# smcconoughey/erpl_monte_carlo_sim

Measured on AMD Instinct MI355X. Metric: Monte Carlo trajectories/sec (whole node) + apogee-match rate, higher is better.
Workload: dtype f64_fast

## Files before the change

erpl_monte_carlo_sim_amd/csrc/erpl_k_config.h:

```cpp
#pragma once

#ifndef ERPL_FAITHFUL
#define ERPL_FAITHFUL 0
#endif
#ifndef ERPL_FAST_F64
#define ERPL_FAST_F64 0
#endif
#ifndef ERPL_FAST_F32
#define ERPL_FAST_F32 0
#endif
#if ERPL_FAITHFUL + ERPL_FAST_F64 + ERPL_FAST_F32 != 1
#error "define exactly one of ERPL_FAITHFUL, ERPL_FAST_F64, ERPL_FAST_F32 to 1 before including erpl_kernels.inc"
#endif

#define ERPL_CAT_(a, b) a##b
#define ERPL_CAT(a, b) ERPL_CAT_(a, b)
#if ERPL_FAITHFUL
typedef double real;
#define ERPL_SUFFIX f64
#elif ERPL_FAST_F64
typedef double real;
#define ERPL_SUFFIX f64f
#else
typedef float real;
#define ERPL_SUFFIX f32
#endif
#define ERPL_LAUNCH_NAME ERPL_CAT(erpl_launch_, ERPL_SUFFIX)

#ifndef ERPL_STAGE_UNROLL
#if ERPL_FAITHFUL
#define ERPL_STAGE_UNROLL 1
#else
#define ERPL_STAGE_UNROLL 4
#endif
#endif
#ifndef ERPL_FLIGHT_MIN_WAVES
#if ERPL_FAITHFUL
#define ERPL_FLIGHT_MIN_WAVES 1
#else
#define ERPL_FLIGHT_MIN_WAVES 2
#endif
#endif
#ifndef ERPL_DENSE_WAVES
#define ERPL_DENSE_WAVES 3
#endif
#ifndef ERPL_SWEEP_CAPPED_WAVES
#define ERPL_SWEEP_CAPPED_WAVES 2
#endif
#ifndef ERPL_RAIL_BLOCK
#define ERPL_RAIL_BLOCK 64
#endif
#ifndef ERPL_HANDOFF_SPEED
#define ERPL_HANDOFF_SPEED 1e6
#endif

#ifndef ERPL_STAMPS
#define ERPL_STAMPS 0
#endif
#if ERPL_STAMPS
#define ERPL_STAMP(acc_, last_)                                                          \
  do {                                                                                   \
    __builtin_amdgcn_sched_barrier(0);                                                   \
    unsigned long long now_;                                                             \
    asm volatile("s_memtime %0\n\ts_waitcnt lgkmcnt(0)" : "=s"(now_)::"memory");          \
    __builtin_amdgcn_sched_barrier(0);                                                   \
    acc_ += now_ - last_;                                                                \
    last_ = now_;                                                                        \
  } while (0)
#else
#define ERPL_STAMP(acc_, last_) do { } while (0)
#endif

namespace {
constexpr bool kFaithful = (ERPL_FAITHFUL != 0);
constexpr int kWave = 64;
struct StampSums { unsigned long long seg[8]; unsigned long long last; };
}
#define ERPL_RARE_BLOCK() asm volatile("")
```

erpl_monte_carlo_sim_amd/csrc/erpl_k_debug.h:

```cpp
namespace {

#if ERPL_FAITHFUL
struct RecordEval {
  real mass, cg, Ixx, Iyy;
  real T, P, rho;
  real vb0, vb1, vb2, vn, mach;
  real alpha, beta;
  real cd, cl, cy, cm, cyaw, cp_dyn;
  real qdyn, thrust, drag, margin;
};
__device__ __forceinline__ void record_eval(const Shared& C, const LaneParams& p, int64_t id, double ts,
                                            const real (&y)[14], RecordEval& e) {
  const ErplScalars<real>& S = *C.S;
  mass_props(S, p, y[13], e.mass, e.cg, e.Ixx, e.Iyy);
  atmosphere(S, y[2], e.T, e.P);
  e.rho = e.P / (S.Rg * e.T);
  WindCache wc;
  wc.lo = 1; wc.hi = 0; wc.x0 = 0;
#pragma unroll
  for (int c = 0; c < 3; ++c) { wc.y0[c] = 0; wc.s[c] = 0; }
  real wv[3];
  wind_at(C, id, y[2], wc, wv);
  const real vr0 = y[3] - wv[0], vr1 = y[4] - wv[1], vr2 = y[5] - wv[2];
  real w = y[6], x = y[7], yy = y[8], z = y[9];
// ... 29 lines not shown
}

__device__ __forceinline__ void lane_params_of(const ErplKArgs& a, const ErplScalars<real>& S, int64_t id, LaneParams& p) {
  const int64_t n = a.n;
  p.dry = (real)a.rocket[0 * n + id]; p.prop = (real)a.rocket[1 * n + id];
  p.thrust = (real)a.motor[0 * n + id]; p.Ae = (real)a.motor[1 * n + id];
  p.mdot = (real)a.motor[2 * n + id]; p.burn = a.motor[3 * n + id];
  lane_params_finish(S, p);
}

__global__ __launch_bounds__(256) void erpl_extract_f64(const ErplKArgs a, const ErplScalars<real> S,
                                                        const double time_offset) {
  __shared__ LdsTables L;
  __shared__ real alt_s[ERPL_MAX_WIND_KNOTS];
  stage_tables(L, alt_s, a.tables, a.alt_grid, a.k_wind);
  const int64_t r = (int64_t)blockIdx.x * blockDim.x + threadIdx.x;
  if (r >= a.traj_cap) return;
  Shared C;
  C.S = &S; C.L = &L; C.alt = alt_s; C.has_wind = a.k_wind > 0; C.motor_kind = a.motor_kind;
  const int64_t id = a.n_traj;
  LaneParams p;
  lane_params_of(a, S, id, p);
  const double* rec = a.traj + r * ERPL_TRAJ_DIM;
  const double ts = rec[0] - time_offset;
  real y[14];
#pragma unroll
  for (int c = 0; c < 14; ++c) y[c] = (real)rec[1 + c];
  double* o = a.summary + r * ERPL_DIAG_DIM;
  {
    const real w = y[6], x = y[7], yy = y[8], z = y[9];
    o[0] = atan2(2 * (w * x + yy * z), 1 - 2 * (x * x + yy * yy));
    const real sinp = 2 * (w * yy - z * x);
    o[1] = (fabs(sinp) >= 1) ? copysign(1.57079632679489661923, sinp) : asin(sinp);
    o[2] = atan2(2 * (w * z + x * yy), 1 - 2 * (yy * yy + z * z));
  }
  RecordEval e;
  record_eval(C, p, id, ts, y, e);
  o[3] = e.cg; o[4] = e.mass; o[5] = e.Ixx; o[6] = e.Iyy; o[7] = e.Iyy;
  o[8] = e.thrust;
  o[9] = e.drag;
  o[10] = e.cd; o[11] = e.cl; o[12] = e.cm;
  o[13] = e.cp_dyn;
  o[14] = e.margin;
  o[15] = e.alpha; o[16] = e.beta;
}
#endif

__global__ __launch_bounds__(256) void ERPL_CAT(erpl_debug_, ERPL_SUFFIX)(const ErplKArgs a, const ErplScalars<real> S,
                                                                         const int what, const int64_t m,
                                                                         const double* __restrict__ in,
                                                                         double* __restrict__ out) {
  __shared__ LdsTables L;
  __shared__ real alt_s[ERPL_MAX_WIND_KNOTS];
  stage_tables(L, alt_s, a.tables, a.alt_grid, a.k_wind);
  const int64_t j = (int64_t)blockIdx.x * blockDim.x + threadIdx.x;
  const int64_t n = a.n;
  if (j >= ((what == ERPL_DBG_RHS_SEQ) ? n : m)) return;
  Shared C;
  C.S = &S; C.L = &L; C.alt = alt_s; C.has_wind = a.k_wind > 0; C.motor_kind = a.motor_kind;
  const int64_t id = j % n;
  LaneParams p;
  p.dry = (real)a.rocket[0 * n + id]; p.prop = (real)a.rocket[1 * n + id];
  p.thrust = (real)a.motor[0 * n + id]; p.Ae = (real)a.motor[1 * n + id];
  p.mdot = (real)a.motor[2 * n + id]; p.burn = a.motor[3 * n + id];
  lane_params_finish(S, p);
  WindCache wc;
  wc.lo = 1; wc.hi = 0; wc.x0 = 0;
#pragma unroll
  for (int c = 0; c < 3; ++c) { wc.y0[c] = 0; wc.s[c] = 0; }
  MachCache mc;
  mach_cache_clear(mc);
  AtmCache ac;
  atm_cache_clear(ac);
#if !ERPL_FAITHFUL
  LaneRec lr;
#if ERPL_FAST_F64
  __shared__ real lane_wind[kLwSlots][kWave];
  lr.lw = &lane_wind[0][threadIdx.x];
  lr.put_wind(wc);
#endif
#endif
  if (what == ERPL_DBG_ATMOSPHERE) {
    const real h = (real)in[j];
    real T, P, rho, g;
#if ERPL_FAITHFUL
    atmosphere(S, h, T, P);
    rho = m_div(P, S.Rg * T);
    g = gravity_at(S, h);
#else
    real rT;
    altitude_tables_reload(C, id, h, wc, ac);
    fast_atmosphere(C, ac, h, T, rT, P);
    rho = (P * S.inv_Rg) * rT;
    const real re = (real)6.371e6;
    const real r = re * m_rcp(re + h);
    g = S.g0 * (r * r);
#endif
    out[0 * m + j] = (double)T; out[1 * m + j] = (double)P; out[2 * m + j] = (double)rho; out[3 * m + j] = (double)g;
  } else if (what == ERPL_DBG_AERO) {
    const real mach = (real)in[0 * m + j], alpha = (real)in[1 * m + j], beta = (real)in[2 * m + j];
    const real pf = (real)in[3 * m + j];
    mach_lookup(C, mach, mc);
    real cd, cl, cy, cm, cyaw;
#if ERPL_FAITHFUL
    real mass, cg, Ixx, Iyy, cp_dyn;
    mass_props(S, p, pf, mass, cg, Ixx, Iyy);
    aero_coefficients(S, mach_rec_of(C, mc), mach, alpha, beta, cg, in[4 * m + j] > 0.0, cd, cl, cy, cm, cyaw, cp_dyn);
#else
    const real mp = p.prop * pf;
    const real cg = (p.dry_cg + mp * S.prop_cg) * m_rcp(p.dry + mp);
    real cma;
    fast_aero(S, mach_rec_of(C, mc), mach, mach * mach, alpha, beta, pf, cg, cd, cl, cy, cma);
    cm = cma * alpha; cyaw = cma * beta;
#endif
    out[0 * m + j] = (double)cd; out[1 * m + j] = (double)cl; out[2 * m + j] = (double)cy;
    out[3 * m + j] = (double)cm; out[4 * m + j] = (double)cyaw;
  } else if (what == ERPL_DBG_MATH) {
    const real x = (real)in[0 * m + j], y = (real)in[1 * m + j];
    real o[ERPL_DBG_MATH_ROWS];
#pragma unroll
    for (int k = 0; k < ERPL_DBG_MATH_ROWS; ++k) o[k] = (real)NAN;
    o[0] = m_rcp(x);
    o[5] = m_exp(x); o[6] = m_pow(x, y); o[7] = m_div(x, y); o[8] = m_atan2(y, x);
    o[14] = m_next_up(x); o[15] = m_sqrt(x);
#if ERPL_FAITHFUL
    o[2] = m_sqrt(x);
#else
    o[1] = m_rsq(x); o[2] = m_sqrt_pos(x);
    o[3] = m_exp2(x, x); o[4] = m_log2(x, x);
    o[9] = m_clamp(x, (real)-1, y);
    {
      const real v2 = m_max(x * x + y * y, (real)1e-30);
      const real r = v2 * m_rsq(v2);
      m_aero_angles(y, x, r, y, m_abs(x), r, x, o[10], o[11]);
#if ERPL_FAST_F64
      o[12] = m_atan2_half<false>(y, x, r, x);
      o[13] = m_atan2_half<true>(y, m_abs(x), r, x);
#endif
    }
#endif
#pragma unroll
    for (int k = 0; k < ERPL_DBG_MATH_ROWS; ++k) out[k * m + j] = (double)o[k];
  } else {
    const int64_t stride = (what == ERPL_DBG_RHS_SEQ) ? n : m;
// ... 21 lines not shown
```

erpl_monte_carlo_sim_amd/csrc/erpl_k_flight.h:

```cpp
namespace {

struct Lane {
#if ERPL_FAST_F64
  real* yl;
#else
  real y[14];
#endif
  double t, t_rail;
  double apogee_t, first_apogee_t, latch_t;
  real apogee, first_apogee;
  real max_speed2, max_coast;
  real cx, cy;
  int64_t id;
  int64_t traj_slot;
  int32_t steps, nrail;
  int32_t mode;
  int32_t stop_steps;
  bool chute, nan_seen, apogee_detected;
};

#if ERPL_FAST_F64
#define LY(ln_, c_) (ln_).yl[((c_) >> 1) * (2 * kWave) + ((c_) & 1)]
#else
#define LY(ln_, c_) (ln_).y[c_]
// ... 27 lines not shown
  s[ERPL_SUM_RANGE * n + i] = sqrt(x * x + yv * yv);
  s[ERPL_SUM_FLIGHT_TIME * n + i] = ln.t - ln.t_rail;
  s[ERPL_SUM_IMPACT_X * n + i] = x;
  s[ERPL_SUM_IMPACT_Y * n + i] = yv;
  s[ERPL_SUM_IMPACT_Z * n + i] = (double)LY(ln, 2);
  s[ERPL_SUM_STEPS * n + i] = (double)ln.steps;
  s[ERPL_SUM_FINAL_VZ * n + i] = (double)LY(ln, 5);
  s[ERPL_SUM_MAX_SPEED * n + i] = (double)m_sqrt(ln.max_speed2);
  a->status[i] = end | (ln.apogee_detected ? ERPL_ST_APOGEE_LATCHED : 0) | (ln.chute ? ERPL_ST_CHUTE : 0) |
                 (ln.nan_seen ? ERPL_ST_NAN : 0);
  ln.mode = kIdle;
}

__device__ __forceinline__ void park_record(Lane& ln, int64_t traj_len, real* rr, double* rd, int32_t* ri, int64_t cap,
                                            unsigned long long e) {
#pragma unroll
  for (int c = 0; c < 14; ++c) rr[c * cap + e] = LY(ln, c);
  rr[14 * cap + e] = ln.apogee; rr[15 * cap + e] = ln.first_apogee; rr[16 * cap + e] = ln.max_speed2;
  rr[17 * cap + e] = ln.max_coast; rr[18 * cap + e] = ln.cx; rr[19 * cap + e] = ln.cy;
  rd[0 * cap + e] = ln.t; rd[1 * cap + e] = ln.t_rail; rd[2 * cap + e] = ln.apogee_t;
  rd[3 * cap + e] = ln.first_apogee_t; rd[4 * cap + e] = ln.latch_t;
  ri[0 * cap + e] = (int32_t)ln.id; ri[1 * cap + e] = ln.steps; ri[2 * cap + e] = ln.nrail;
  ri[3 * cap + e] = (ln.mode << 8) | (ln.chute ? kRecChute : 0) | (ln.nan_seen ? kRecNanSeen : 0) |
                    (ln.apogee_detected ? kRecApogee : 0);
  ri[4 * cap + e] = (int32_t)traj_len;
  ln.mode = kIdle;
}

__device__ __forceinline__ real rk4_combine(real y, real dt_sixth, real acc, real k4) { return y + dt_sixth * (acc + k4); }

template <typename T> __device__ __forceinline__ bool m_finite(T x) { return (x - x) == (T)0; }

#if ERPL_FAST_F64
constexpr int kFlightBlock = kWave;
constexpr bool kStepsAcrossLoop = true;
#else
constexpr int kFlightBlock = 256;
constexpr bool kStepsAcrossLoop = false;
#endif
template <bool TRAJ, int SPEC, int MINW>
__global__ __launch_bounds__(kFlightBlock, MINW) void ERPL_CAT(erpl_flight_, ERPL_SUFFIX)(const ErplKArgs a, const ErplScalars<real> S) {
  {
    const unsigned long long n_in0 = (a.phase == 0) ? (unsigned long long)a.n : a.qcnt[a.phase];
    const unsigned long long taken0 = (a.phase == 0) ? 0ull : a.qhead[a.phase];
    if ((unsigned long long)blockIdx.x * blockDim.x >= n_in0 - (taken0 < n_in0 ? taken0 : n_in0)) return;
  }
  __shared__ LdsTables L;
#if ERPL_FAST_F64
  extern __shared__ double erpl_dyn_lds[];
  real* const alt_s = (real*)erpl_dyn_lds;
#else
  __shared__ real alt_s[ERPL_MAX_WIND_KNOTS];
#endif
  stage_tables(L, alt_s, a.tables, a.alt_grid, a.k_wind);
  Shared C;
  C.S = &S;
  C.L = &L;
  C.alt = alt_s;
  C.has_wind = (SPEC < 0) ? (a.k_wind > 0) : ((SPEC & 1) != 0);
  C.motor_kind = (SPEC < 0) ? a.motor_kind : ((SPEC & 2) ? (int)ERPL_MOTOR_SOLID : (int)ERPL_MOTOR_LIQUID);
  const double dt = a.dt_flight, max_time = a.max_time;
  const real dt_sixth = S.dt_sixth, half_dt = S.half_dt, full_dt = S.dt_flight;
  const int refill_threshold = a.refill_threshold;
  const int chunk_steps = a.chunk_steps;
  const int adopt_lanes = TRAJ ? 0 : a.adopt_lanes;
  const bool stop_at_apogee = (a.flags & ERPL_FLAG_STOP_AT_APOGEE) != 0;
  const bool traj_fast_forward = TRAJ && (a.flags & ERPL_FLAG_CAPTURE_POSITION_ONLY) != 0;
  const int lane = threadIdx.x & (kWave - 1);

  Lane ln;
  ln.mode = kIdle; ln.id = -1; ln.traj_slot = -1;
  LaneParams p;
  WindCache wc;
  MachCache mc;
  mach_cache_clear(mc);
  AtmCache ac;
  atm_cache_clear(ac);
  LaneRec lr;
#if ERPL_FAST_F64
  __shared__ __attribute__((aligned(16))) real lane_y[7][kWave][2];
  ln.yl = &lane_y[0][threadIdx.x][0];
  __shared__ real lane_wind[kLwSlots][kWave];
  lr.lw = &lane_wind[0][threadIdx.x];
#endif
#if ERPL_FAST_F32
  __shared__ double t_store[2][256];
  double* const tl = &t_store[0][threadIdx.x];
  double* const bl = &t_store[1][threadIdx.x];
#endif
  int64_t traj_len = 0;
  bool queue_empty = false;
  unsigned long long wave_iters = 0, steps_done = 0;
  StampSums ss;
#pragma unroll
  for (int i = 0; i < 8; ++i) ss.seg[i] = 0;
  ss.last = 0;
#if ERPL_STAMPS
  asm volatile("s_memtime %0\n\ts_waitcnt lgkmcnt(0)" : "=s"(ss.last)::"memory");
#endif

#if ERPL_FAST_F64
  bool extreme = false;
#endif
  for (;;) {
#if ERPL_FAST_F64
    {
      const bool hx = (ln.mode == kPhysics) && extreme;
      const unsigned long long xm = __ballot(hx);
      if (xm != 0ull) {
        ColdArgs ca = cold_args();
        unsigned long long base = 0;
        if (lane == 0) base = atomicAdd(ca->ext_cnt, (unsigned long long)__popcll(xm));
        base = __shfl(base, 0);
        if (hx) {
          const int rank = __builtin_amdgcn_mbcnt_hi((unsigned)(xm >> 32), __builtin_amdgcn_mbcnt_lo((unsigned)xm, 0));
          park_record(ln, traj_len, (real*)ca->ext_r, ca->ext_d, ca->ext_i, ca->res_cap, base + (unsigned long long)rank);
        }
      }
      extreme = false;
    }
#endif
    {
      bool thin = false;
      if (adopt_lanes > 0 && queue_empty) thin = __popcll(__ballot(ln.mode == kPhysics)) <= adopt_lanes;
      const bool need = (ln.mode == kPhysics) && (thin || ln.steps >= ln.stop_steps);
      const unsigned long long dm = __ballot(need);
      if (dm != 0ull) {
        ColdArgs ca = cold_args();
        const int ph = ca->phase;
        const int64_t cap = ca->res_cap;
        unsigned long long base = 0;
        if (lane == 0) base = atomicAdd(&ca->qcnt[ph + 1], (unsigned long long)__popcll(dm));
        base = __shfl(base, 0);
        if (need) {
          const int rank = __builtin_amdgcn_mbcnt_hi((unsigned)(dm >> 32), __builtin_amdgcn_mbcnt_lo((unsigned)dm, 0));
          const unsigned long long e = base + (unsigned long long)rank;
          park_record(ln, traj_len, (real*)ca->res_r[(ph + 1) & 1], ca->res_d[(ph + 1) & 1], ca->res_i[(ph + 1) & 1], cap, e);
        }
        if (adopt_lanes > 0) {
          __builtin_amdgcn_fence(__ATOMIC_RELEASE, "agent");
          if (need) {
            const int rank = __builtin_amdgcn_mbcnt_hi((unsigned)(dm >> 32), __builtin_amdgcn_mbcnt_lo((unsigned)dm, 0));
            __hip_atomic_store(&ca->res_i[(ph + 1) & 1][5 * cap + (int64_t)(base + (unsigned long long)rank)], ph + 1,
                               __ATOMIC_RELAXED, __HIP_MEMORY_SCOPE_AGENT);
          }
        }
      }
    }
    const unsigned long long idle = __ballot(ln.mode == kIdle);
    const int n_idle = __popcll(idle);
// ... 20 lines not shown
        unsigned long long got = 0;
        if (lane == 0) {
          const unsigned long long r = __hip_atomic_load(&ca->qcnt[src], __ATOMIC_RELAXED, __HIP_MEMORY_SCOPE_AGENT);
          unsigned long long h = __hip_atomic_load(&ca->qhead[src], __ATOMIC_RELAXED, __HIP_MEMORY_SCOPE_AGENT);
          if (h < r) {
            const unsigned long long want = (r - h < (unsigned long long)n_idle) ? r - h : (unsigned long long)n_idle;
            if (__hip_atomic_compare_exchange_strong(&ca->qhead[src], &h, h + want, __ATOMIC_RELAXED, __ATOMIC_RELAXED,
                                                     __HIP_MEMORY_SCOPE_AGENT)) { base = h; got = want; }
          }
        }
        base = __shfl(base, 0);
        n_in = base + __shfl(got, 0);
      }
      if (ln.mode == kIdle) {
        const int rank = __builtin_amdgcn_mbcnt_hi((unsigned)(idle >> 32), __builtin_amdgcn_mbcnt_lo((unsigned)idle, 0));
        const unsigned long long e = base + (unsigned long long)rank;
        if (e < n_in) {
          bool lost = false;
          if (adopt) {
            const int limit = ca->adopt_spin;
            int spins = 0;
            lost = limit < 0;
            while (!lost && __hip_atomic_load(&ri[5 * cap + e], __ATOMIC_RELAXED, __HIP_MEMORY_SCOPE_AGENT) != src) {
              __builtin_amdgcn_s_sleep(8);
              if (++spins > limit) lost = true;
            }
            if (lost) atomicAdd(&ca->counters[3], 1ull);
            __builtin_amdgcn_fence(__ATOMIC_ACQUIRE, "agent");
          }
          if (!lost) {
#pragma unroll
          for (int c = 0; c < 14; ++c) LY(ln, c) = rr[c * cap + e];
          ln.apogee = rr[14 * cap + e]; ln.first_apogee = rr[15 * cap + e]; ln.max_speed2 = (real)rr[16 * cap + e];
          ln.max_coast = (real)rr[17 * cap + e]; ln.cx = (real)rr[18 * cap + e]; ln.cy = (real)rr[19 * cap + e];
          ln.t = rd[0 * cap + e]; ln.t_rail = rd[1 * cap + e]; ln.apogee_t = rd[2 * cap + e];
          ln.first_apogee_t = rd[3 * cap + e]; ln.latch_t = rd[4 * cap + e];
          const int64_t id = ri[0 * cap + e];
          ln.id = id; ln.steps = ri[1 * cap + e]; ln.nrail = ri[2 * cap + e];
          const int fl = ri[3 * cap + e];
          ln.mode = fl >> 8;
          ln.chute = (fl & kRecChute) != 0; ln.nan_seen = (fl & kRecNanSeen) != 0;
          ln.apogee_detected = (fl & kRecApogee) != 0;
          ln.stop_steps = (chunk_steps > 0) ? ln.steps + chunk_steps : 0x7fffffff;
          p.dry = (real)rocket[0 * n + id]; p.prop = (real)rocket[1 * n + id];
          p.thrust = (real)motor[0 * n + id]; p.Ae = (real)motor[1 * n + id];
          p.mdot = (real)motor[2 * n + id]; p.burn = motor[3 * n + id];
#if ERPL_FAST_F32
          *bl = p.burn;
#endif
          lane_params_finish(S, p);
          wc.lo = 1; wc.hi = 0; wc.x0 = 0;
#pragma unroll
          for (int c = 0; c < 3; ++c) { wc.y0[c] = 0; wc.s[c] = 0; }
          lr.put_wind(wc);
          mach_cache_clear(mc);
          atm_cache_clear(ac);
          if (TRAJ) {
            ln.traj_slot = -1; traj_len = ri[4 * cap + e];
            for (int64_t m = 0; m < ca->n_traj; ++m) if (ca->traj_ids[m] == id) ln.traj_slot = m;
          }
          if (fl & kRecFresh) {
            traj_record<TRAJ>(ln, traj_len, false);
            if (!(ln.t < max_time)) {
              if (TRAJ && ln.traj_slot >= 0) ca->traj_len[ln.traj_slot] = traj_len;
              lane_finish(ln, ERPL_END_MAX_TIME);
            }
          }
          }
        }
      }
    }
    const unsigned long long phys = __ballot(ln.mode == kPhysics);
    if (phys == 0ull) {
      if (__ballot(ln.mode == kCoast) == 0ull) { if (queue_empty) break; else continue; }
      for (int burst = 0; burst < 256; ++burst) {
        if (ln.mode == kCoast) {
          LY(ln, 0) = rk4_combine(LY(ln, 0), dt_sixth, ln.cx, (real)0);
          LY(ln, 1) = rk4_combine(LY(ln, 1), dt_sixth, ln.cy, (real)0);
          ln.t += dt;
          ln.steps++;
          if (!(ln.t < max_time)) lane_finish(ln, ERPL_END_MAX_TIME);
        }
        if (__ballot(ln.mode == kCoast) == 0ull) break;
      }
      continue;
    }
    bool ended, nonfinite, alt_nan, latch_now, coast_out;
    ERPL_STAMP(ss.seg[0], ss.last);
#if ERPL_FAST_F32
    if (ln.mode == kPhysics) *tl = ln.t;
#endif
    if (kStepsAcrossLoop && ln.mode == kPhysics) steps_done -= (unsigned long long)ln.steps;
    do {
    ++wave_iters;
    ended = false; nonfinite = false; alt_nan = false; latch_now = false; coast_out = false;
#if ERPL_FAST_F64
    extreme = false;
#endif
    if (!ERPL_FAST_F32 && ln.mode == kCoast) {
      LY(ln, 0) = rk4_combine(LY(ln, 0), dt_sixth, ln.cx, (real)0);
      LY(ln, 1) = rk4_combine(LY(ln, 1), dt_sixth, ln.cy, (real)0);
      ln.t += dt;
      ln.steps++;
      if (!(ln.t < max_time)) lane_finish(ln, ERPL_END_MAX_TIME);
    }
    if (ln.mode == kPhysics) {
      real k[14], ys[14], acc[14];
#pragma unroll
      for (int c = 0; c < 14; ++c) { ys[c] = (real)LY(ln, c); acc[c] = 0; }
#if !ERPL_FAITHFUL
      int gates;
      real gate_t[3] = {0, 0, 0};
      {
#if ERPL_FAST_F32
        const double tb = *tl, burn = *bl;
#else
        const double tb = ln.t, burn = p.burn;
#endif
        const double th = tb + 0.5 * dt, tf = tb + dt;
        gates = ((tb <= burn) ? 1 : 0) | ((th <= burn) ? 2 : 0) | ((tf <= burn) ? 4 : 0);
        gates = (tb >= 0.0) ? gates : 0;
        if (C.motor_kind == ERPL_MOTOR_SOLID) { gate_t[0] = (real)tb; gate_t[1] = (real)th; gate_t[2] = (real)tf; }
      }
#if ERPL_FAST_F32
      asm volatile("" ::: "memory");
#endif
#endif
#pragma unroll ERPL_STAGE_UNROLL
      for (int stage = 0; stage < 4; ++stage) {
#if ERPL_FAITHFUL
        const double ts = (stage == 0) ? ln.t : ((stage == 3) ? ln.t + dt : ln.t + 0.5 * dt);
        rocket_dynamics(C, p, ln.id, wc, mc, ac, ln.chute, ts, ys, k, ss);
#else
        const int gi = (stage == 0) ? 0 : ((stage == 3) ? 2 : 1);
        rocket_dynamics_at<true>(C, p, ln.id, wc, mc, ac, ln.chute, 0.0, ((gates >> gi) & 1) != 0, gate_t[gi], ys, k, ss, lr);
#endif
        const real wgt = (stage == 0 || stage == 3) ? (real)1 : (real)2;
        const real adv = (stage == 2) ? full_dt : half_dt;
        if (stage < 3) {
#pragma unroll
          for (int c = 0; c < 14; ++c) {
            acc[c] = (stage == 0) ? k[c] : acc[c] + wgt * k[c];
            ys[c] = LY(ln, c) + adv * k[c];
          }
        }
        ERPL_STAMP(ss.seg[5], ss.last);
      }
      real yn[14];
#pragma unroll
      for (int c = 0; c < 14; ++c) yn[c] = rk4_combine(LY(ln, c), dt_sixth, acc[c], k[c]);
      {
        const real n2 = ((yn[6] * yn[6] + yn[7] * yn[7]) + yn[8] * yn[8]) + yn[9] * yn[9];
#if ERPL_FAITHFUL
        const real nrm = m_sqrt(n2);
        if (nrm > (real)1e-12) { yn[6] /= nrm; yn[7] /= nrm; yn[8] /= nrm; yn[9] /= nrm; }
        else { yn[6] = 1; yn[7] = 0; yn[8] = 0; yn[9] = 0; }
#else
        const real r = m_rsq(n2);
        yn[6] *= r; yn[7] *= r; yn[8] *= r; yn[9] *= r;
        if (!(n2 > (real)1e-24)) { ERPL_RARE_BLOCK(); yn[6] = 1; yn[7] = 0; yn[8] = 0; yn[9] = 0; }
#endif
      }
#pragma unroll
      for (int c = 0; c < 14; ++c) LY(ln, c) = yn[c];
#if ERPL_FAST_F32
      const double t_now = *tl + dt;
      *tl = t_now;
#else
      ln.t += dt;
      const double t_now = ln.t;
#endif
      ln.steps++;
      if (!kStepsAcrossLoop) ++steps_done;
      ERPL_STAMP(ss.seg[6], ss.last);
      const real alt = yn[2], vz = yn[5];
      alt_nan = m_isnan(alt);
      {
        const bool upd = !ln.nan_seen && (alt_nan || alt > ln.apogee);
        ln.apogee = upd ? alt : ln.apogee;
        ln.apogee_t = upd ? t_now : ln.apogee_t;
        ln.nan_seen = ln.nan_seen || alt_nan;
      }
      {
        const real sp2 = (real)((yn[3] * yn[3] + yn[4] * yn[4]) + vz * vz);
        ln.max_speed2 = (sp2 > ln.max_speed2) ? sp2 : ln.max_speed2;
#if ERPL_FAST_F64
        extreme = (sp2 > (real)(ERPL_HANDOFF_SPEED * ERPL_HANDOFF_SPEED)) || (alt < (real)-1e5);
#endif
// ... 62 lines not shown
          const bool burning = (pfc > 0) && (ln.t <= burn_time);
          bool fin = true;
#pragma unroll
          for (int c = 6; c < 13; ++c) fin = fin && m_finite(LY(ln, c));
          if (!burning && fin) {
            const real vx = (real)LY(ln, 3), vy = (real)LY(ln, 4);
            ln.cx = ((vx + 2 * vx) + 2 * vx) + vx;
            ln.cy = ((vy + 2 * vy) + 2 * vy) + vy;
#if !ERPL_FAST_F32
            const real x0 = LY(ln, 0), y0 = LY(ln, 1);
            const real x1 = rk4_combine(x0, dt_sixth, ln.cx, (real)0), y1 = rk4_combine(y0, dt_sixth, ln.cy, (real)0);
            const bool still = ((x1 == x0) || (m_isnan(x1) && m_isnan(x0))) && ((y1 == y0) || (m_isnan(y1) && m_isnan(y0)));
            if (still) {
              ColdArgs cc = cold_args();
              if (TRAJ) {
                traj_record<TRAJ>(ln, traj_len, false);
                while (ln.t < max_time) { ln.t += dt; ln.steps++; if (ln.t < max_time) traj_record<TRAJ>(ln, traj_len, false); }
              } else if (ln.nrail < cc->n_coast) {
                ln.t = cc->tables->coast_t[ln.nrail];
                ln.steps = cc->tables->coast_steps[ln.nrail];
              } else {
                while (ln.t < max_time) { ln.t += dt; ln.steps++; }
              }
              end = ERPL_END_MAX_TIME;
            } else if (!TRAJ) {
              ln.mode = kCoast;
            }
#else
            if (!TRAJ) {
            ColdArgs cc = cold_args();
            double tf = ln.t;
            int32_t total = ln.steps;
            if (ln.nrail < cc->n_coast) { tf = cc->tables->coast_t[ln.nrail]; total = cc->tables->coast_steps[ln.nrail]; }
            else { while (tf < max_time) { tf += dt; total++; } }
            const real m = (real)(total - ln.steps);
            LY(ln, 0) = LY(ln, 0) + m * (dt_sixth * ln.cx);
            LY(ln, 1) = LY(ln, 1) + m * (dt_sixth * ln.cy);
            ln.t = tf; ln.steps = total;
            end = ERPL_END_MAX_TIME;
            }
#endif
          }
        }
      }
      traj_record<TRAJ>(ln, traj_len, end >= 0);
      if (end >= 0) {
        if (TRAJ && ln.traj_slot >= 0) cold_args()->traj_len[ln.traj_slot] = traj_len;
        lane_finish(ln, end);
      }
      }
    }
  }
  ColdArgs ca = cold_args();
#if ERPL_STAMPS
  if (lane == 0) {
#pragma unroll
    for (int i = 0; i < 8; ++i) atomicAdd(&ca->counters[8 + i], ss.seg[i]);
  }
#endif
  if (lane == 0) atomicAdd(&ca->counters[2], wave_iters);
  for (int off = 32; off > 0; off >>= 1) steps_done += __shfl_down(steps_done, off);
  if (lane == 0) atomicAdd(&ca->counters[1], steps_done);
}

}
```

erpl_monte_carlo_sim_amd/csrc/erpl_k_lookup.h:

```cpp
namespace {

enum { kIdle = 0, kPhysics = 1, kCoast = 2 };
enum { kRecChute = 1, kRecNanSeen = 2, kRecApogee = 4, kRecFresh = 8 };

typedef const ErplKArgs __attribute__((address_space(4))) * ColdArgs;
__device__ __forceinline__ ColdArgs cold_args() {
  ColdArgs p = (ColdArgs)__builtin_amdgcn_kernarg_segment_ptr();
  asm volatile("" : "+s"(p));
  return p;
}

#if ERPL_FAST_F64
constexpr int kMachRec = ERPL_MACH_REC + 2;
constexpr int kMachRecs = ERPL_MAX_UNION_KNOTS + 2;
constexpr int kMachEmpty = ERPL_MAX_UNION_KNOTS + 1;
#else
constexpr int kMachRec = ERPL_MACH_REC;
constexpr int kMachRecs = ERPL_MAX_UNION_KNOTS + 1;
#endif
struct LdsTables {
  alignas(16) real mach_rec[kMachRecs * kMachRec];
  alignas(16) real atm[ERPL_ATM_LAYERS * ERPL_ATM_REC];
  real union_knots[ERPL_MAX_UNION_KNOTS];
  real curve_t[ERPL_MAX_CURVE_KNOTS];
  real curve_f[ERPL_MAX_CURVE_KNOTS];
  real alt_map[2];
};

__device__ __forceinline__ void stage_tables(LdsTables& L, real* alt, const ErplTables* __restrict__ T,
                                             const double* __restrict__ alt_grid, int k_wind) {
  const int tid = threadIdx.x, nt = blockDim.x;
#if ERPL_FAST_F64
  {
    const int n_union = T->n_union;
    for (int i = tid; i < kMachRecs * kMachRec; i += nt) {
      const int idx = i / kMachRec, k = i - idx * kMachRec;
      real v;
      if (idx > n_union) v = (k == 0) ? (real)1 : (real)0;
      else if (k == 0) v = (idx == 0) ? (real)-INFINITY : (real)T->union_knots[idx - 1];
      else if (k == 1) v = (idx == n_union) ? (real)INFINITY : (real)T->union_knots[idx];
      else v = (real)T->mach_rec[idx * ERPL_MACH_REC + (k - 2)];
      L.mach_rec[i] = v;
    }
  }
#else
  for (int i = tid; i < (ERPL_MAX_UNION_KNOTS + 1) * ERPL_MACH_REC; i += nt) L.mach_rec[i] = (real)T->mach_rec[i];
#endif
  for (int i = tid; i < ERPL_MAX_UNION_KNOTS; i += nt) L.union_knots[i] = (real)T->union_knots[i];
  for (int i = tid; i < ERPL_MAX_CURVE_KNOTS; i += nt) {
    L.curve_t[i] = (real)T->curve_t[i];
    L.curve_f[i] = (real)T->curve_f[i];
  }
  for (int i = tid; i < k_wind; i += nt) alt[i] = (real)alt_grid[i];
  if (tid == 0) {
    const real a0 = (k_wind > 0) ? (real)alt_grid[0] : (real)0;
    const real span = (k_wind > 1) ? (real)alt_grid[k_wind - 1] - a0 : (real)0;
    L.alt_map[0] = a0;
    L.alt_map[1] = (span > 0) ? (real)(k_wind - 1) / span : (real)0;
  }
  for (int i = tid; i < ERPL_ATM_LAYERS * ERPL_ATM_REC; i += nt) L.atm[i] = (real)T->atm_rec[i];
  __syncthreads();
}

struct LaneParams {
  real dry, prop;
  real thrust, Ae, mdot;
  double burn;
  real dry_cg;
  real pfr0, inv_abs_pfr;
};

__device__ __forceinline__ void lane_params_finish(const ErplScalars<real>& S, LaneParams& p) {
  p.dry_cg = p.dry * S.cg_dry;
  p.pfr0 = -p.mdot / p.prop;
  p.inv_abs_pfr = (p.pfr0 != 0) ? (real)1 / ((p.pfr0 < 0) ? -p.pfr0 : p.pfr0) : (real)INFINITY;
}

struct WindCache {
  real lo, hi, x0;
// ... 139 lines not shown
}
#else
struct MachCache {
  real lo, hi;
  real rec[ERPL_MACH_REC];
  int idx;
};
__device__ __forceinline__ void mach_cache_clear(MachCache& mc) {
  mc.lo = 1; mc.hi = 0; mc.idx = 0;
#pragma unroll
  for (int k = 0; k < ERPL_MACH_REC; ++k) mc.rec[k] = 0;
}
__device__ __forceinline__ const real* mach_rec_of(const Shared&, const MachCache& mc) { return mc.rec; }
__device__ __forceinline__ bool mach_inside(const Shared&, const MachCache& mc, real mach) { return mach >= mc.lo && mach < mc.hi; }

__device__ __forceinline__ void mach_reload(const Shared& C, real mach, MachCache& mc) {
  const LdsTables& L = *C.L;
  const int n_union = cold_args()->n_union;
  int idx = mc.idx + ((mach >= mc.hi) ? 1 : -1);
  idx = (idx < 0) ? 0 : ((idx > n_union) ? n_union : idx);
  real lo = (idx == 0) ? -INFINITY : L.union_knots[idx - 1];
  real hi = (idx == n_union) ? INFINITY : L.union_knots[idx];
  if (!(mach >= lo && mach < hi)) {
    idx = 0;
    for (int j = 0; j < n_union; ++j) idx += (mach >= L.union_knots[j]) ? 1 : 0;
    lo = (idx == 0) ? -INFINITY : L.union_knots[idx - 1];
    hi = (idx == n_union) ? INFINITY : L.union_knots[idx];
  }
  mc.lo = lo; mc.hi = hi; mc.idx = idx;
#pragma unroll
  for (int k = 0; k < ERPL_MACH_REC; ++k) mc.rec[k] = L.mach_rec[idx * ERPL_MACH_REC + k];
}
#endif

__device__ __forceinline__ void mach_lookup(const Shared& C, real mach, MachCache& mc) {
  if (!mach_inside(C, mc, mach)) mach_reload(C, mach, mc);
}

__device__ __forceinline__ real solid_curve(const Shared& C, real tt, real mult) {
  const LdsTables& L = *C.L;
  const int n_curve = cold_args()->n_curve;
  int j = 0;
  for (int k = 0; k < n_curve; ++k) j += (tt >= L.curve_t[k]) ? 1 : 0;
  if (j == 0) return L.curve_f[0] * mult;
  if (j == n_curve) return L.curve_f[n_curve - 1] * mult;
  const real x0 = L.curve_t[j - 1], x1 = L.curve_t[j];
  const real y0 = L.curve_f[j - 1] * mult, y1 = L.curve_f[j] * mult;
  return m_div(y1 - y0, x1 - x0) * (tt - x0) + y0;
}

#if ERPL_FAITHFUL
struct AtmCache { real lo, hi, alo, ahi; };
__device__ __forceinline__ void atm_cache_clear(AtmCache& ac) { ac.lo = 1; ac.hi = 0; ac.alo = 1; ac.ahi = 0; }
struct LaneRec { __device__ __forceinline__ void put_wind(const WindCache&) const {} };
#else
struct AtmCache {
  real lo, hi;
  real alo, ahi;
#if ERPL_FAST_F64
  int ro;
#else
  real r[10];
#endif
};
__device__ __forceinline__ void atm_cache_clear(AtmCache& ac) {
  ac.lo = 1; ac.hi = 0; ac.alo = 1; ac.ahi = 0;
#if ERPL_FAST_F64
  ac.ro = 0;
#endif
}

__device__ __forceinline__ void altitude_tables_reload(const Shared& C, int64_t id, real h, WindCache& wc, AtmCache& ac) {
  const ErplScalars<real>& S = *C.S;
  if (!ERPL_FAST_F32 || !(h >= ac.alo && h < ac.ahi)) {
    const int li = ((h > S.h_tropo) ? 1 : 0) + ((h > S.h_strat) ? 1 : 0) + ((h > (real)25000.0) ? 1 : 0) +
                   ((h > (real)32000.0) ? 1 : 0);
#if ERPL_FAST_F64
    ac.ro = li * kAtmRecBytes;
#else
#pragma unroll
    for (int k = 0; k < 10; ++k) ac.r[k] = C.L->atm[li * ERPL_ATM_REC + k];
#endif
    const real llo = (li == 0) ? -INFINITY : ((li == 1) ? S.h_tropo : ((li == 2) ? S.h_strat : ((li == 3) ? (real)25000.0 : (real)32000.0)));
    const real lhi = (li == 0) ? S.h_tropo : ((li == 1) ? S.h_strat : ((li == 2) ? (real)25000.0 : ((li == 3) ? (real)32000.0 : INFINITY)));
    ac.alo = (llo > -INFINITY) ? m_next_up(llo) : llo;
    ac.ahi = (lhi < INFINITY) ? m_next_up(lhi) : lhi;
  }
  real lo = ac.alo, hi = ac.ahi;
  if (C.has_wind) {
    if (!(h >= wc.lo && h < wc.hi)) wind_reload(C, id, h, wc);
    lo = (wc.lo > lo) ? wc.lo : lo;
    hi = (wc.hi < hi) ? wc.hi : hi;
  }
  ac.lo = lo; ac.hi = hi;
}

enum { kLwLo = 0, kLwHi, kLwX0, kLwY0, kLwS = kLwY0 + 3, kLwSlots = kLwS + 3 };
struct LaneRec {
#if ERPL_FAST_F64
  real* lw;
  __device__ __forceinline__ void fence() const { asm volatile("" ::: "memory"); }
  __device__ __forceinline__ void wind_bounds(WindCache& wc) const { wc.lo = lw[kLwLo * kWave]; wc.hi = lw[kLwHi * kWave]; }
  __device__ __forceinline__ void wind(WindCache& wc) const {
    wc.x0 = lw[kLwX0 * kWave];
#pragma unroll
    for (int c = 0; c < 3; ++c) { wc.y0[c] = lw[(kLwY0 + c) * kWave]; wc.s[c] = lw[(kLwS + c) * kWave]; }
  }
  __device__ __forceinline__ void put_wind(const WindCache& wc) const {
    lw[kLwLo * kWave] = wc.lo; lw[kLwHi * kWave] = wc.hi; lw[kLwX0 * kWave] = wc.x0;
#pragma unroll
    for (int c = 0; c < 3; ++c) { lw[(kLwY0 + c) * kWave] = wc.y0[c]; lw[(kLwS + c) * kWave] = wc.s[c]; }
  }
#else
  __device__ __forceinline__ void fence() const {}
  __device__ __forceinline__ void wind_bounds(WindCache&) const {}
  __device__ __forceinline__ void wind(WindCache&) const {}
  __device__ __forceinline__ void put_wind(const WindCache&) const {}
#endif
};
#endif

}
```

erpl_monte_carlo_sim_amd/csrc/erpl_k_rhs_fast.h:

```cpp
namespace {

__device__ __forceinline__ void fast_atmosphere(const Shared& C, const AtmCache& ac, real h, real& T, real& rT, real& P) {
#if ERPL_FAST_F64
  real r[10];
  {
    const RealPair* q = lds_record(C.L->atm, ac.ro);
#pragma unroll
    for (int k = 0; k < 5; ++k) { const RealPair v = q[k]; r[2 * k] = v.x; r[2 * k + 1] = v.y; }
  }
#else
  (void)C;
  const real* r = ac.r;
#endif
  const real aT = r[0], bT = r[1], Tlo = r[2], Thi = r[3];
  const real invTref = r[4], eL = r[5], href = r[6], eH = r[7], eM = r[8], pbase = r[9];
  T = m_clamp(bT + aT * h, Tlo, Thi);
  rT = m_rcp(T);
  P = pbase * m_exp2(eL * m_log2(T * invTref, h) + (h - href) * (eH + eM * rT), h);
}

__device__ __forceinline__ void fast_aero(const ErplScalars<real>& S, const real* rec, real mach, real mach2,
                                          real alpha, real beta, real pf, real cg, real& cd, real& cl, real& cy,
                                          real& cma) {
  const real mq = m_clamp(mach, (real)0, kBig);
  const real dm = mq - rec[0];
  const real cd0 = rec[2] * dm + rec[1];
  const real cda = rec[4] * dm + rec[3];
  const real cps = rec[7] * (mq - rec[5]) + rec[6];
  cd = cd0 + cda * (alpha * alpha);
  cd = (pf > 0) ? cd : cd * S.power_off;
  const real abs_alpha = m_abs(alpha);
  const real cl_alpha = S.two_pi_AR_cos * m_rcp((real)2 + m_sqrt_pos((real)4 + S.AR_over_cos2 * m_abs((real)1 - mach2)));
  cy = cl_alpha * beta;
  {
    const real over = m_max(abs_alpha - S.stall_angle, (real)0);
    const real sf = m_max((real)1 - over * S.inv_stall_span, (real)0);
    cd *= (real)1 + ((real)0.5 * over) * S.inv_stall_span;
    cy *= sf;
    cl = cl_alpha * m_copysign(m_clamp(abs_alpha, (real)-1, S.stall_angle) * sf, alpha);
  }
  const real sm = (S.cp_location + cps) - cg;
  cma = -cl_alpha * sm;
}

template <bool GATED>
__device__ __forceinline__ void rocket_dynamics_at(const Shared& C, LaneParams& p, int64_t id,
                                                   WindCache& wc, MachCache& mc, AtmCache& ac, bool& chute, double t,
                                                   bool gate_le_burn, real gate_t,
                                                   const real (&y)[14], real (&dy)[14], StampSums& ss,
                                                   const LaneRec lr) {
  const ErplScalars<real>& S = *C.S;
  const real h = y[2];
  if (!(h >= ac.lo && h < ac.hi)) {
    ERPL_RARE_BLOCK();
    lr.wind_bounds(wc);
    lr.wind(wc);
    altitude_tables_reload(C, id, h, wc, ac);
    lr.put_wind(wc);
  }
  lr.fence();
  lr.wind(wc);
  real wv[3] = {0, 0, 0};
  if (C.has_wind) {
    const real d = m_clamp(h, -kBig, kBig) - wc.x0;
    wv[0] = wc.s[0] * d + wc.y0[0]; wv[1] = wc.s[1] * d + wc.y0[1]; wv[2] = wc.s[2] * d + wc.y0[2];
  }
  ERPL_STAMP(ss.seg[1], ss.last);
  const real pf = m_max(y[13], (real)0);
  real q0, q1, q2, q3;
  {
    const real r = m_rsq((((y[6] * y[6] + y[7] * y[7]) + y[8] * y[8]) + y[9] * y[9]) * (real)0.5);
    q0 = y[6] * r; q1 = y[7] * r; q2 = y[8] * r; q3 = y[9] * r;
  }
  const real q11 = q1 * q1, q22 = q2 * q2, q33 = q3 * q3;
  const real R00 = ((real)1 - q22) - q33, R01 = q1 * q2 - q0 * q3, R02 = q1 * q3 + q0 * q2;
  const real R10 = q1 * q2 + q0 * q3, R11 = ((real)1 - q11) - q33, R12 = q2 * q3 - q0 * q1;
  const real R20 = q1 * q3 - q0 * q2, R21 = q2 * q3 + q0 * q1, R22 = ((real)1 - q11) - q22;
  const real mp = p.prop * pf;
  const real mass = p.dry + mp;
  const real rm = m_rcp(mass);
  const real cg = (p.dry_cg + mp * S.prop_cg) * rm;
  const real Ixx = S.Ixx_dry + mp * S.dq2;
  const real dcg = S.prop_cg - cg;
  const real Iyy = S.Iyy_dry + mp * (S.third + dcg * dcg);
  const real ri = m_rcp(Iyy);
  real T, rT, P;
  fast_atmosphere(C, ac, h, T, rT, P);
  const real vr0 = y[3] - wv[0], vr1 = y[4] - wv[1], vr2 = y[5] - wv[2];
  const real vb0 = (R00 * vr0 + R10 * vr1) + R20 * vr2;
  const real vb1 = (R01 * vr0 + R11 * vr1) + R21 * vr2;
  const real vb2 = (R02 * vr0 + R12 * vr1) + R22 * vr2;
  const real vn2 = (vr0 * vr0 + vr1 * vr1) + vr2 * vr2;
  const real mach2 = (vn2 * rT) * (real)(1.0 / (1.4 * 287.053));
  const real qdyn = (S.q_of_PM2 * P) * mach2;
  const bool burning = (pf > 0) && (GATED ? gate_le_burn : (t >= 0.0 && t <= p.burn));
  real thrust;
  if (C.motor_kind == ERPL_MOTOR_SOLID) {
    thrust = burning ? solid_curve(C, GATED ? gate_t : (real)t, p.thrust) + p.Ae * ((real)101325.0 - P) : (real)0;
  } else {
    thrust = burning ? p.thrust - p.Ae * P : (real)0;
  }
  real fb0 = thrust, fb1 = 0, fb2 = 0, mb1 = 0, mb2 = 0;
  ERPL_STAMP(ss.seg[2], ss.last);
  if (h <= S.chute_alt) { if (!chute && y[5] < 0) chute = true; }
  if (chute) {
    const real rs2 = (vb0 * vb0 + vb1 * vb1) + vb2 * vb2;
    const real rs = m_sqrt(rs2);
    if (rs > 0) {
      const real rho = (P * S.inv_Rg) * rT;
      const real kc = -(rho * rs2) * S.chute_k * m_rcp(rs);
      fb0 += kc * vb0; fb1 += kc * vb1; fb2 += kc * vb2;
    }
  }
  if (!chute && qdyn > 0) {
// ... 68 lines not shown
```

Baseline: 6.288 million.

## Replace altitude-crossing reload with incremental wind-segment stepping and LDS layer ranges

On the fast-f64 path, an altitude-crossing handler now keeps the wind knot index per lane in LDS and steps it by one on each crossing, with grid and binary-search fallbacks, instead of a full table reload. Atmosphere layer bounds are precomputed into LDS once per block, which drops the alo/ahi fields from the per-lane cache. The per-lane LDS wind record now holds an int index slot instead of the lower bound, and the wind values are only read back from LDS when not crossing (or when the trajectory readback template flag is set). The aim is to shorten the rare but divergent crossing block and reduce register pressure, at the cost of extra complexity. A counting mode for crossings is also added for profiling.

Result: no change. 6.317 million (median of 6 runs) (+0.5%).

```diff
diff --git a/erpl_monte_carlo_sim_amd/csrc/erpl_k_config.h b/erpl_monte_carlo_sim_amd/csrc/erpl_k_config.h
--- a/erpl_monte_carlo_sim_amd/csrc/erpl_k_config.h
+++ b/erpl_monte_carlo_sim_amd/csrc/erpl_k_config.h
@@ -57,7 +57,18 @@
 #ifndef ERPL_STAMPS
 #define ERPL_STAMPS 0
 #endif
-#if ERPL_STAMPS
+#if ERPL_STAMPS == 2
+#define ERPL_COUNT_CROSSING(ss_, miss_)                                                              \
+  do {                                                                                               \
+    const bool first_ = (int)(threadIdx.x & (kWave - 1)) == __ffsll((long long)__ballot(true)) - 1;  \
+    const unsigned long long any_ = __ballot(miss_);                                                 \
+    (ss_).seg[0] += (first_ & (any_ != 0ull)) ? 1ull : 0ull;                                         \
+    (ss_).seg[1] += (miss_) ? 1ull : 0ull;                                                           \
+  } while (0)
+#else
+#define ERPL_COUNT_CROSSING(ss_, miss_) do { } while (0)
+#endif
+#if ERPL_STAMPS == 1
 #define ERPL_STAMP(acc_, last_)                                                          \
   do {                                                                                   \
     __builtin_amdgcn_sched_barrier(0);                                                   \
diff --git a/erpl_monte_carlo_sim_amd/csrc/erpl_k_debug.h b/erpl_monte_carlo_sim_amd/csrc/erpl_k_debug.h
--- a/erpl_monte_carlo_sim_amd/csrc/erpl_k_debug.h
+++ b/erpl_monte_carlo_sim_amd/csrc/erpl_k_debug.h
@@ -105,6 +105,9 @@
                                                                          double* __restrict__ out) {
   __shared__ LdsTables L;
   __shared__ real alt_s[ERPL_MAX_WIND_KNOTS];
+#if ERPL_FAST_F64
+  stage_layer_ranges(L, S);
+#endif
   stage_tables(L, alt_s, a.tables, a.alt_grid, a.k_wind);
   const int64_t j = (int64_t)blockIdx.x * blockDim.x + threadIdx.x;
   const int64_t n = a.n;
@@ -128,9 +131,9 @@
 #if !ERPL_FAITHFUL
   LaneRec lr;
 #if ERPL_FAST_F64
-  __shared__ real lane_wind[kLwSlots][kWave];
+  __shared__ LaneSlot lane_wind[kLwSlots][kWave];
   lr.lw = &lane_wind[0][threadIdx.x];
-  lr.put_wind(wc);
+  lr.reset();
 #endif
 #endif
   if (what == ERPL_DBG_ATMOSPHERE) {
@@ -142,7 +145,11 @@
     g = gravity_at(S, h);
 #else
     real rT;
+#if ERPL_FAST_F64
+    altitude_crossing(C, id, h, lr, wc, ac);
+#else
     altitude_tables_reload(C, id, h, wc, ac);
+#endif
     fast_atmosphere(C, ac, h, T, rT, P);
     rho = (P * S.inv_Rg) * rT;
     const real re = (real)6.371e6;
diff --git a/erpl_monte_carlo_sim_amd/csrc/erpl_k_flight.h b/erpl_monte_carlo_sim_amd/csrc/erpl_k_flight.h
--- a/erpl_monte_carlo_sim_amd/csrc/erpl_k_flight.h
+++ b/erpl_monte_carlo_sim_amd/csrc/erpl_k_flight.h
@@ -103,6 +103,9 @@
 #else
   __shared__ real alt_s[ERPL_MAX_WIND_KNOTS];
 #endif
+#if ERPL_FAST_F64
+  stage_layer_ranges(L, S);
+#endif
   stage_tables(L, alt_s, a.tables, a.alt_grid, a.k_wind);
   Shared C;
   C.S = &S;
@@ -131,7 +134,7 @@
 #if ERPL_FAST_F64
   __shared__ __attribute__((aligned(16))) real lane_y[7][kWave][2];
   ln.yl = &lane_y[0][threadIdx.x][0];
-  __shared__ real lane_wind[kLwSlots][kWave];
+  __shared__ LaneSlot lane_wind[kLwSlots][kWave];
   lr.lw = &lane_wind[0][threadIdx.x];
 #endif
 #if ERPL_FAST_F32
@@ -146,7 +149,7 @@
 #pragma unroll
   for (int i = 0; i < 8; ++i) ss.seg[i] = 0;
   ss.last = 0;
-#if ERPL_STAMPS
+#if ERPL_STAMPS == 1
   asm volatile("s_memtime %0\n\ts_waitcnt lgkmcnt(0)" : "=s"(ss.last)::"memory");
 #endif
 
@@ -273,7 +276,7 @@
           wc.lo = 1; wc.hi = 0; wc.x0 = 0;
 #pragma unroll
           for (int c = 0; c < 3; ++c) { wc.y0[c] = 0; wc.s[c] = 0; }
-          lr.put_wind(wc);
+          lr.reset();
           mach_cache_clear(mc);
           atm_cache_clear(ac);
           if (TRAJ) {
@@ -354,7 +357,7 @@
         rocket_dynamics(C, p, ln.id, wc, mc, ac, ln.chute, ts, ys, k, ss);
 #else
         const int gi = (stage == 0) ? 0 : ((stage == 3) ? 2 : 1);
-        rocket_dynamics_at<true>(C, p, ln.id, wc, mc, ac, ln.chute, 0.0, ((gates >> gi) & 1) != 0, gate_t[gi], ys, k, ss, lr);
+        rocket_dynamics_at<true, TRAJ>(C, p, ln.id, wc, mc, ac, ln.chute, 0.0, ((gates >> gi) & 1) != 0, gate_t[gi], ys, k, ss, lr);
 #endif
         const real wgt = (stage == 0 || stage == 3) ? (real)1 : (real)2;
         const real adv = (stage == 2) ? full_dt : half_dt;
@@ -523,6 +526,9 @@
     }
   }
   ColdArgs ca = cold_args();
+#if ERPL_STAMPS == 2
+  for (int off = 32; off > 0; off >>= 1) { ss.seg[0] += __shfl_down(ss.seg[0], off); ss.seg[1] += __shfl_down(ss.seg[1], off); }
+#endif
 #if ERPL_STAMPS
   if (lane == 0) {
 #pragma unroll
diff --git a/erpl_monte_carlo_sim_amd/csrc/erpl_k_lookup.h b/erpl_monte_carlo_sim_amd/csrc/erpl_k_lookup.h
--- a/erpl_monte_carlo_sim_amd/csrc/erpl_k_lookup.h
+++ b/erpl_monte_carlo_sim_amd/csrc/erpl_k_lookup.h
@@ -25,6 +25,9 @@
   real curve_t[ERPL_MAX_CURVE_KNOTS];
   real curve_f[ERPL_MAX_CURVE_KNOTS];
   real alt_map[2];
+#if ERPL_FAST_F64
+  alignas(16) real atm_range[ERPL_ATM_LAYERS * 2];
+#endif
 };
 
 __device__ __forceinline__ void stage_tables(LdsTables& L, real* alt, const ErplTables* __restrict__ T,
@@ -270,39 +273,43 @@
 #if ERPL_FAITHFUL
 struct AtmCache { real lo, hi, alo, ahi; };
 __device__ __forceinline__ void atm_cache_clear(AtmCache& ac) { ac.lo = 1; ac.hi = 0; ac.alo = 1; ac.ahi = 0; }
-struct LaneRec { __device__ __forceinline__ void put_wind(const WindCache&) const {} };
+struct LaneRec { __device__ __forceinline__ void reset() const {} };
 #else
 struct AtmCache {
   real lo, hi;
+#if ERPL_FAST_F64
+  int ro;
+#else
   real alo, ahi;
-#if ERPL_FAST_F64
-  int ro;
-#else
   real r[10];
 #endif
 };
 __device__ __forceinline__ void atm_cache_clear(AtmCache& ac) {
-  ac.lo = 1; ac.hi = 0; ac.alo = 1; ac.ahi = 0;
+  ac.lo = 1; ac.hi = 0;
 #if ERPL_FAST_F64
   ac.ro = 0;
-#endif
-}
-
+#else
+  ac.alo = 1; ac.ahi = 0;
+#endif
+}
+
+__device__ __forceinline__ int atm_layer_of(const ErplScalars<real>& S, real h) {
+  return ((h > S.h_tropo) ? 1 : 0) + ((h > S.h_strat) ? 1 : 0) + ((h > (real)25000.0) ? 1 : 0) + ((h > (real)32000.0) ? 1 : 0);
+}
+__device__ __forceinline__ void atm_layer_range(const ErplScalars<real>& S, int li, real& alo, real& ahi) {
+  const real llo = (li == 0) ? -INFINITY : ((li == 1) ? S.h_tropo : ((li == 2) ? S.h_strat : ((li == 3) ? (real)25000.0 : (real)32000.0)));
+  const real lhi = (li == 0) ? S.h_tropo : ((li == 1) ? S.h_strat : ((li == 2) ? (real)25000.0 : ((li == 3) ? (real)32000.0 : INFINITY)));
+  alo = (llo > -INFINITY) ? m_next_up(llo) : llo;
+  ahi = (lhi < INFINITY) ? m_next_up(lhi) : lhi;
+}
+
+#if ERPL_FAST_F32
 __device__ __forceinline__ void altitude_tables_reload(const Shared& C, int64_t id, real h, WindCache& wc, AtmCache& ac) {
-  const ErplScalars<real>& S = *C.S;
-  if (!ERPL_FAST_F32 || !(h >= ac.alo && h < ac.ahi)) {
-    const int li = ((h > S.h_tropo) ? 1 : 0) + ((h > S.h_strat) ? 1 : 0) + ((h > (real)25000.0) ? 1 : 0) +
-                   ((h > (real)32000.0) ? 1 : 0);
-#if ERPL_FAST_F64
-    ac.ro = li * kAtmRecBytes;
-#else
+  if (!(h >= ac.alo && h < ac.ahi)) {
+    const int li = atm_layer_of(*C.S, h);
 #pragma unroll
     for (int k = 0; k < 10; ++k) ac.r[k] = C.L->atm[li * ERPL_ATM_REC + k];
-#endif
-    const real llo = (li == 0) ? -INFINITY : ((li == 1) ? S.h_tropo : ((li == 2) ? S.h_strat : ((li == 3) ? (real)25000.0 : (real)32000.0)));
-    const real lhi = (li == 0) ? S.h_tropo : ((li == 1) ? S.h_strat : ((li == 2) ? (real)25000.0 : ((li == 3) ? (real)32000.0 : INFINITY)));
-    ac.alo = (llo > -INFINITY) ? m_next_up(llo) : llo;
-    ac.ahi = (lhi < INFINITY) ? m_next_up(lhi) : lhi;
+    atm_layer_range(*C.S, li, ac.alo, ac.ahi);
   }
   real lo = ac.alo, hi = ac.ahi;
   if (C.has_wind) {
@@ -312,30 +319,106 @@
   }
   ac.lo = lo; ac.hi = hi;
 }
-
-enum { kLwLo = 0, kLwHi, kLwX0, kLwY0, kLwS = kLwY0 + 3, kLwSlots = kLwS + 3 };
+#endif
+
+union LaneSlot { real v; int j; };
+enum { kLwJ = 0, kLwHi, kLwX0, kLwY0, kLwS = kLwY0 + 3, kLwSlots = kLwS + 3 };
 struct LaneRec {
 #if ERPL_FAST_F64
-  real* lw;
+  LaneSlot* lw;
   __device__ __forceinline__ void fence() const { asm volatile("" ::: "memory"); }
-  __device__ __forceinline__ void wind_bounds(WindCache& wc) const { wc.lo = lw[kLwLo * kWave]; wc.hi = lw[kLwHi * kWave]; }
+  __device__ __forceinline__ void reset() const {
+#pragma unroll
+    for (int k = kLwHi; k < kLwSlots; ++k) lw[k * kWave].v = (real)0;
+    lw[kLwJ * kWave].j = 0;
+  }
   __device__ __forceinline__ void wind(WindCache& wc) const {
-    wc.x0 = lw[kLwX0 * kWave];
-#pragma unroll
-    for (int c = 0; c < 3; ++c) { wc.y0[c] = lw[(kLwY0 + c) * kWave]; wc.s[c] = lw[(kLwS + c) * kWave]; }
-  }
-  __device__ __forceinline__ void put_wind(const WindCache& wc) const {
-    lw[kLwLo * kWave] = wc.lo; lw[kLwHi * kWave] = wc.hi; lw[kLwX0 * kWave] = wc.x0;
-#pragma unroll
-    for (int c = 0; c < 3; ++c) { lw[(kLwY0 + c) * kWave] = wc.y0[c]; lw[(kLwS + c) * kWave] = wc.s[c]; }
+    wc.x0 = lw[kLwX0 * kWave].v;
+#pragma unroll
+    for (int c = 0; c < 3; ++c) { wc.y0[c] = lw[(kLwY0 + c) * kWave].v; wc.s[c] = lw[(kLwS + c) * kWave].v; }
+  }
+  __device__ __forceinline__ void put_wind(const WindCache& wc, int j) const {
+    lw[kLwHi * kWave].v = wc.hi; lw[kLwX0 * kWave].v = wc.x0;
+#pragma unroll
+    for (int c = 0; c < 3; ++c) { lw[(kLwY0 + c) * kWave].v = wc.y0[c]; lw[(kLwS + c) * kWave].v = wc.s[c]; }
+    lw[kLwJ * kWave].j = j;
   }
 #else
   __device__ __forceinline__ void fence() const {}
-  __device__ __forceinline__ void wind_bounds(WindCache&) const {}
+  __device__ __forceinline__ void reset() const {}
   __device__ __forceinline__ void wind(WindCache&) const {}
-  __device__ __forceinline__ void put_wind(const WindCache&) const {}
-#endif
-};
-#endif
-
-}
+#endif
+};
+#endif
+
+#if ERPL_FAST_F64
+__device__ __forceinline__ void stage_layer_ranges(LdsTables& L, const ErplScalars<real>& S) {
+  if (threadIdx.x < ERPL_ATM_LAYERS) atm_layer_range(S, (int)threadIdx.x, L.atm_range[2 * threadIdx.x], L.atm_range[2 * threadIdx.x + 1]);
+}
+
+__device__ __forceinline__ void altitude_crossing(const Shared& C, int64_t id, real h, const LaneRec lr, WindCache& wc,
+                                                  AtmCache& ac) {
+  const LdsTables& L = *C.L;
+  const real whi = lr.lw[kLwHi * kWave].v;
+  int j = lr.lw[kLwJ * kWave].j;
+  ColdArgs ca = cold_args();
+  const int k_wind = ca->k_wind;
+  const real* __restrict__ wind = (const real*)ca->wind;
+  const uint32_t n = (uint32_t)ca->n;
+  const int li = atm_layer_of(*C.S, h);
+  const RealPair range = *lds_record(L.atm_range, li * (int)sizeof(RealPair));
+  ac.ro = li * kAtmRecBytes;
+  real lo = range.x, hi = range.y;
+  if (C.has_wind) {
+    j += (h >= whi) ? 1 : -1;
+    j = (j < 0) ? 0 : ((j > k_wind) ? k_wind : j);
+    real below = (j > 0) ? C.alt[j - 1] : -INFINITY;
+    real above = (j < k_wind) ? C.alt[j] : INFINITY;
+    if (!(below <= h && h < above)) {
+      ERPL_RARE_BLOCK();
+      const real g = (h - L.alt_map[0]) * L.alt_map[1];
+      j = (g >= 0) ? ((g < (real)k_wind) ? (int)g + 1 : k_wind) : 0;
+      below = (j > 0) ? C.alt[j - 1] : -INFINITY;
+      above = (j < k_wind) ? C.alt[j] : INFINITY;
+    }
+    if (!(below <= h && h < above)) {
+      ERPL_RARE_BLOCK();
+      int bl = 0, bh = k_wind;
+      while (bl < bh) {
+        int mid = (bl + bh) >> 1;
+        if (C.alt[mid] <= h) bl = mid + 1; else bh = mid;
+      }
+      j = bl;
+      below = (j > 0) ? C.alt[j - 1] : -INFINITY;
+      above = (j < k_wind) ? C.alt[j] : INFINITY;
+    }
+    const int r3 = ((j == k_wind) ? k_wind - 1 : ((j > 0) ? j - 1 : 0)) * 3;
+    const real* __restrict__ row = wind + ((uint64_t)(uint32_t)r3 * (uint64_t)n + (uint64_t)id);
+    if (j == 0 || j == k_wind) {
+      wc.x0 = (j == 0) ? above : below;
+      wc.lo = (j == 0) ? -INFINITY : wc.x0;
+      wc.hi = (j == 0) ? wc.x0 : INFINITY;
+#pragma unroll
+      for (int c = 0; c < 3; ++c) { wc.y0[c] = *row; row += n; wc.s[c] = 0; }
+    } else {
+      const real x0 = below, x1 = above;
+      wc.x0 = x0; wc.lo = x0; wc.hi = x1;
+      const real dx = x1 - x0;
+      real v[6];
+#pragma unroll
+      for (int c = 0; c < 6; ++c) { v[c] = *row; row += n; }
+#pragma unroll
+      for (int c = 0; c < 6; ++c) asm volatile("" : "+v"(v[c]));
+      const real rdx = m_rcp(dx);
+#pragma unroll
+      for (int c = 0; c < 3; ++c) { wc.y0[c] = v[c]; wc.s[c] = (v[3 + c] - v[c]) * rdx; }
+    }
+    lr.put_wind(wc, j);
+    lo = (wc.lo > lo) ? wc.lo : lo;
+    hi = (wc.hi < hi) ? wc.hi : hi;
+  }
+  ac.lo = lo; ac.hi = hi;
+}
+#endif
+
+}
diff --git a/erpl_monte_carlo_sim_amd/csrc/erpl_k_rhs_fast.h b/erpl_monte_carlo_sim_amd/csrc/erpl_k_rhs_fast.h
--- a/erpl_monte_carlo_sim_amd/csrc/erpl_k_rhs_fast.h
+++ b/erpl_monte_carlo_sim_amd/csrc/erpl_k_rhs_fast.h
@@ -43,7 +43,7 @@
   cma = -cl_alpha * sm;
 }
 
-template <bool GATED>
+template <bool GATED, bool READBACK = false>
 __device__ __forceinline__ void rocket_dynamics_at(const Shared& C, LaneParams& p, int64_t id,
                                                    WindCache& wc, MachCache& mc, AtmCache& ac, bool& chute, double t,
                                                    bool gate_le_burn, real gate_t,
@@ -51,15 +51,23 @@
                                                    const LaneRec lr) {
   const ErplScalars<real>& S = *C.S;
   const real h = y[2];
-  if (!(h >= ac.lo && h < ac.hi)) {
+  const bool crossing = !(h >= ac.lo && h < ac.hi);
+  ERPL_COUNT_CROSSING(ss, crossing);
+#if ERPL_FAST_F64
+  lr.fence();
+  if (crossing) {
     ERPL_RARE_BLOCK();
-    lr.wind_bounds(wc);
+    altitude_crossing(C, id, h, lr, wc, ac);
+    if (READBACK) { lr.fence(); lr.wind(wc); }
+  } else {
     lr.wind(wc);
+  }
+#else
+  if (crossing) {
+    ERPL_RARE_BLOCK();
     altitude_tables_reload(C, id, h, wc, ac);
-    lr.put_wind(wc);
   }
-  lr.fence();
-  lr.wind(wc);
+#endif
   real wv[3] = {0, 0, 0};
   if (C.has_wind) {
     const real d = m_clamp(h, -kBig, kBig) - wc.x0;
```
